# aidanmrli/rwm-pt-pytorch

Hardware: AMD Instinct MI355X
Metric: chain-MH-steps/sec (higher is better)
Workload: dtype f32; 1 GPU; BASELINE configs[2]: PT-RWM HIP, RoughCarpet dim=30 modes[-15,0,15], Normal proposal 2.38^2/dim, 32 geometric temps 1->0.01, swap_every=10, 65536 ladders per GPU; dim=30, temps=32, ladders_per_gpu=65536, mh_steps_per_launch=2000, swap_every=10, swap_mode=exchange, swap_order=sequential, rng=Philox4x32-10 in-kernel, world_size=1

## Files before the change

### rwm-pt-pytorch_amd/csrc/kernel.h

```cpp
#pragma once
#include <cstddef>
#include <type_traits>

#include "flow.h"
#include "philox.h"
#include "proposals.h"
#include "targets.h"

namespace ptrwm {

#ifndef PTRWM_BLOCK_THREADS
#define PTRWM_BLOCK_THREADS 256
#endif
constexpr int kBlockThreads = PTRWM_BLOCK_THREADS;
constexpr int kWavesPerBlock = kBlockThreads / 64;
struct StepLdsWords {
  static constexpr int kSwapWords = 3;
  static constexpr int kParkedInts = 3;
  static constexpr int kExtraPerThread = kSwapWords + kParkedInts + 2;
  static constexpr int kStreamSlabs = 2;
  static constexpr int kStreamStatPerThread = 5;
  static constexpr unsigned kVoteBytes = 16u;
  static constexpr unsigned kFlowLdsUnit = 8u;
  static constexpr int kFlowIntsPerThread = 4;
  static constexpr int kFlowUp = 2, kFlowDown = 3;
  static constexpr unsigned flow_bytes(int threads) { return (unsigned)(threads * kFlowIntsPerThread) * 4u; }
  static constexpr int floats_per_thread(int dp, bool stream) { return (stream ? kStreamSlabs * (dp + kStreamStatPerThread) : dp) + kExtraPerThread; }
  static constexpr unsigned bytes(int threads, int dp, bool stream, bool wide) { return (unsigned)(threads * floats_per_thread(dp, stream)) * 4u + (wide ? kVoteBytes : 0u); }
};
template <int DP, bool STREAM = false>
struct StepLds : StepLdsWords {
  static constexpr int kWaveFloats = 64 * floats_per_thread(DP, STREAM);
  static constexpr int kSlabFloats = 64 * DP;
  static constexpr int kSlabVectorsPerLane = (kSlabFloats + 255) / 256;
  static constexpr int s_l(int gt) { return STREAM ? kStreamSlabs * kSlabFloats : gt * DP; }
  static constexpr int parked(int gt) { return STREAM ? s_l(64) + kSwapWords * 64 : gt * (DP + kSwapWords); }
  static constexpr int sq_jump(int gt) { return STREAM ? s_l(64) + (kSwapWords + kParkedInts) * 64 : gt * (DP + (kSwapWords + kParkedInts)); }
  static constexpr int vote(int gt) { return gt * (DP + kExtraPerThread); }
  static constexpr int kSu = 1, kLanded = 2, kParked = kSwapWords, kVote = kExtraPerThread;
  static constexpr int kSwapCount = 1, kLastEvent = 2, kSqJump = kParkedInts;
  static constexpr int kZoneFloats = 64 * kStreamStatPerThread;
  static constexpr int zone(int slab) { return s_l(64) + 64 * kExtraPerThread + slab * kZoneFloats; }
  static constexpr int kZoneLogp = 0, kZoneSqJump = 64, kZoneAccept = 64 + 2 * 64;
  static constexpr int moments(bool wide, int gt) { return wide ? gt * (DP + kExtraPerThread) + (int)(kVoteBytes / 4u) : kBlockThreads * (DP + kExtraPerThread); }
  __device__ __forceinline__ static double *moments_region(float *s_dyn, bool wide, int gt, int wave, int stride) {
    return reinterpret_cast<double *>(s_dyn + moments(wide, gt)) + (wide ? 0 : wave * stride);
  }
  __device__ __forceinline__ static int *flow_region(float *s_dyn, bool wide, int wave, unsigned flow_lds) {
    return reinterpret_cast<int *>(s_dyn) + (int)flow_lds * (int)(kFlowLdsUnit / 4u) + (wide ? 0 : wave * (64 * kFlowIntsPerThread));
  }
  static constexpr unsigned bytes(int threads, bool wide) { return StepLdsWords::bytes(threads, DP, STREAM, wide); }
  static constexpr int kHeadWaveWords = normal_blocks(DP) * kHeadBlockSlots * kHeadSlotWords;
  static constexpr bool kHeadsFit = !STREAM && kHeadWaveWords <= 64 * (DP + kSwapWords) && kWaveFloats % kHeadSlotWords == 0;
  static constexpr int heads(bool wide, int wave) { return wave * (wide ? kHeadWaveWords : kWaveFloats); }
};
namespace lds_check {
using C = StepLds<30>;
using S = StepLds<30, true>;
static_assert(C::s_l(256) == 256 * 30 && C::parked(256) == C::s_l(256) + C::kParked * 256 &&
                  C::sq_jump(256) == C::parked(256) + C::kSqJump * 256 && C::vote(256) == C::sq_jump(256) + 2 * 256 &&
                  C::vote(256) == C::s_l(256) + C::kVote * 256 && C::moments(true, 256) * 4 == (int)C::bytes(256, true) &&
                  C::moments(false, 64) * 4 == (int)C::bytes(kBlockThreads, false) && C::kWaveFloats == C::vote(64) && 0 < C::kSu &&
                  C::kSu < C::kLanded && C::kLanded < C::kParked && 0 < C::kSwapCount && C::kSwapCount < C::kLastEvent && C::kLastEvent < C::kSqJump,
              "classic layout: rows, swap scratch, parked ints, squared-jump doubles, vote word, moments regions: disjoint, in this order");
static_assert(S::s_l(64) == 2 * S::kSlabFloats && S::parked(64) == S::s_l(64) + 3 * 64 && S::sq_jump(64) == S::parked(64) + 3 * 64 &&
                  S::zone(0) == S::sq_jump(64) + 2 * 64 && S::zone(1) == S::zone(0) + S::kZoneFloats &&
                  S::zone(1) + S::kZoneFloats == S::kWaveFloats && S::kZoneSqJump == S::kZoneLogp + 64 &&
                  S::kZoneAccept == S::kZoneSqJump + 2 * 64 && S::kZoneAccept + 2 * 64 == S::kZoneFloats,
              "streaming layout: two slabs, swap scratch, parked words, two landing zones of three arrays");
template <int DP>
constexpr bool aligned(bool ok = true) {
  using A = StepLds<DP>;
  using B = StepLds<DP, true>;
  for (int gt = 64; gt <= 256; gt += 64) ok = ok && A::sq_jump(gt) % 2 == 0 && A::moments(true, gt) % 2 == 0 && A::moments(false, gt) % 2 == 0;
  for (int z = 0; z < 2; ++z) ok = ok && B::zone(z) % 4 == 0 && (B::zone(z) + B::kZoneSqJump) % 4 == 0 && (B::zone(z) + B::kZoneAccept) % 4 == 0;
  return ok && A::kWaveFloats % 4 == 0 && B::kWaveFloats % 4 == 0 && B::kSlabFloats % 4 == 0 && B::sq_jump(64) % 2 == 0;
}
static_assert(aligned<2>() && aligned<3>() && aligned<5>() && aligned<9>() && aligned<29>() && aligned<30>() && aligned<50>() && aligned<64>(), "alignment");
static_assert(C::bytes(256, false) == 38912u && S::bytes(256, false) == 79872u && C::bytes(256, true) == 38928u, "LDS bytes, as before the layout had a name");
static_assert(C::kHeadsFit && C::kHeadWaveWords == 2048 && C::heads(false, 3) + C::kHeadWaveWords <= 3 * C::kWaveFloats + C::parked(64) &&
                  C::heads(true, 3) + C::kHeadWaveWords <= C::parked(256) && C::heads(true, 1) + C::kHeadWaveWords <= C::parked(128) &&
                  !StepLds<8>::kHeadsFit && !S::kHeadsFit,
              "parked heads: 16-byte slots over the rows and the swap scratch of the wave's group, below the parked words; width 8 has no room");
static_assert(0 < C::kFlowUp && C::kFlowUp < C::kFlowDown && C::kFlowDown < C::kFlowIntsPerThread && C::flow_bytes(256) == 4096u &&
                  C::flow_bytes(kBlockThreads) == (unsigned)kWavesPerBlock * 64u * C::kFlowIntsPerThread * 4u,
              "flow region: two word buffers, up visits, down visits, one region per group; nothing of it in a launch without flow");
}

constexpr int kNoStepInLaunch = (1 << 16) + 1;
struct FullArgs {
  const float *__restrict__ ext_prop;
  const float *__restrict__ ext_u;
  const float *__restrict__ ext_swap_u;
  float *__restrict__ trace;
  float *__restrict__ trace_logp;
  unsigned char *__restrict__ accept_flags;
  long long trace_chains;
  int trace_every;
  int mom_every;
  unsigned steps_to_trace : 17;
  unsigned trace_temps : 9;
  unsigned steps_to_mom : 17;
  unsigned mom_temps : 9;
  unsigned mom_chain : 1;
  double *__restrict__ mom_sum;
  double *__restrict__ mom_sum_sq;
  double *__restrict__ mom_sum_logp;
  long long *__restrict__ mom_count;
  int *__restrict__ flow_walker;
  long long *__restrict__ flow_round_trips;
  long long *__restrict__ flow_up;
  long long *__restrict__ flow_down;
};

typedef const __attribute__((address_space(4))) FullArgs *kargs_full_ptr;

struct KArgs {
  float *__restrict__ state;
  float *__restrict__ logp;
  const float *__restrict__ beta;
  const float *__restrict__ temp_scale;
  long long *__restrict__ n_accept;
  double *__restrict__ sq_jump;
  long long *__restrict__ swap_accept;
  long long *__restrict__ last_swap_ordinal;
  long long n_chains, chain_offset, step0;
  long long first_swap_event;
  int n_steps;
  int burn_left;
  int n_temps, dim, swap_every, swap_mode, swap_order, chains_per_wave;
  int steps_to_swap;
  unsigned k0, k1;
  unsigned full_mom_steps : 17;
  unsigned full_flow_lds : 15;
  TParams tp;
  PParams pp;
  FullArgs full;
};
static_assert(sizeof(FullArgs) == 136 && sizeof(KArgs) == 392 && offsetof(KArgs, tp) == 144, "the kernel arguments keep their size: see FullArgs");
static_assert(PTRWM_MAX_TEMPS < (1 << 9) && kNoStepInLaunch < (1 << 17) && 160u * 1024u / StepLdsWords::kFlowLdsUnit < (1u << 15), "FullArgs bitfield widths");
__host__ __device__ constexpr int ext_raw_per_step(int proposal_kind, int dim) { return dim + (proposal_kind == PTRWM_PROPOSAL_UNIFORM_RADIUS ? 1 : 0); }

__device__ __forceinline__ float swap_log_prob(float bj, float bk, float lj, float lk) {
  return sub_rn(sub_rn(add_rn(mul_rn(bj, lk), mul_rn(bk, lj)), mul_rn(bj, lj)), mul_rn(bk, lk));
}

__device__ __forceinline__ bool swap_accept_test(float u, float log_prob) {
  const float threshold = (log_prob >= 0.0f) ? 1.0f : hw_exp(log_prob);
  return u < threshold;
}

__device__ __forceinline__ bool mh_accept(float beta_t, float lp_new, float lp, float u_acc) {
  const float ratio = mul_rn(beta_t, sub_rn(lp_new, lp));
  return (ratio > 0.0f) || (u_acc < hw_exp(ratio));
}

__device__ __forceinline__ bool swap_pair_plain(int T, int t, float db, float lp, float us) {
  const bool last = t >= T - 1;
  const float u = last ? 0.5f : us;
  const float d = last ? 1.0f : db;
  const float inside = mul_rn(u, sub_rn(1.0f, u));
  return add_rn(__builtin_fminf(inside, d), mul_rn(lp, 0.0f)) > 0.0f;
}
__device__ __forceinline__ bool ladder_votes_plain(bool mine, int first_lane, int lanes_per_ladder) {
  const unsigned long long against = __builtin_amdgcn_ballot_w64(!mine);
  const unsigned long long ladder = (lanes_per_ladder >= 64 ? ~0ull : ((1ull << lanes_per_ladder) - 1ull)) << first_lane;
  return (against & ladder) == 0ull;
}

template <class Sync>
__device__ __forceinline__ bool wide_ladder_votes_plain(int *word, bool mine, int stamp, Sync sync) {
  if (!mine) *word = stamp;
  sync();
  return *word != stamp;
}

__device__ __forceinline__ float swap_uniform_ext(const float *__restrict__ ext_swap_u, long long event, long long n_chains,
                                                  long long chain, int T, int t) {
  return (t < T - 1) ? ext_swap_u[(event * n_chains + chain) * (T - 1) + t] : 2.0f;
}
__device__ __forceinline__ float swap_uniform_philox(uint32_t c0hi, uint32_t c1, uint32_t c2, uint32_t c3, uint32_t k0, uint32_t k1) {
  const u32x4 r = philox4x32_10(c0hi, c1, c2, c3, k0, k1);
  return u01(r.x);
}

#define PTRWM_SWAP_SCAN_PAIR(OK, IK, LK, LANDED_J, CAR_L, CAR_I) \
  do {                                                           \
    (LANDED_J) = (OK) ? (IK) : (CAR_I);                          \
    (CAR_L) = (OK) ? (CAR_L) : (LK);                             \
    (CAR_I) = (OK) ? (CAR_I) : (IK);                             \
  } while (0)

template <class Sync>
__device__ __forceinline__ void swap_decide(int T, int t, int base, int slot, int swap_mode, int swap_order, int par,
                                            const float *__restrict__ beta, float beta_t, float us, const float *s_l,
                                            float *s_u, int *landed, float &my_l, int &src, bool &pair_acc, Sync sync,
                                            bool plain) {
  if (swap_order == PTRWM_ORDER_SEQUENTIAL) {
    if (swap_mode == PTRWM_SWAP_EXCHANGE) {
      const bool has_k = t < T - 1;
      const float db = has_k ? sub_rn(beta_t, beta[t + 1]) : 1.0f;
      float car_l = s_l[base];
      int car_i = base;
      if (plain) {
        const float lk = s_l[has_k ? slot + 1 : slot];
        s_u[slot] = fmaf(-hw_ln(us), __builtin_amdgcn_rcpf(db), lk);
        sync();
#pragma unroll 2
        for (int j = 0; j < T - 1; ++j) {
          const int ik = base + j + 1;
          const float lkj = s_l[ik];
          const bool ok = car_l < s_u[base + j];
          PTRWM_SWAP_SCAN_PAIR(ok, ik, lkj, landed[base + j], car_l, car_i);
        }
      } else {
#pragma unroll 2
        for (int j = 0; j < T - 1; ++j) {
          const float lk = s_l[base + j + 1];
          const float u = s_u[base + j];
          const float bj = beta[j], bk = beta[j + 1];
          const bool ok = swap_accept_test(u, swap_log_prob(bj, bk, car_l, lk));
          const int ik = base + j + 1;
          PTRWM_SWAP_SCAN_PAIR(ok, ik, lk, landed[base + j], car_l, car_i);
        }
      }
      landed[base + T - 1] = car_i;
      src = landed[base + t];
      my_l = s_l[src];
      pair_acc = (t < T - 1) && (src == base + t + 1);
    } else {
      if (t < T - 1) {
        const float lk = s_l[slot + 1];
        const bool ok = swap_accept_test(us, swap_log_prob(beta_t, beta[t + 1], my_l, lk));
        if (ok) {
          my_l = lk;
          src = slot + 1;
        }
        pair_acc = ok;
      }
    }
  } else {
    const bool lower = ((t & 1) == par);
    const int partner_t = lower ? t + 1 : t - 1;
    const bool valid = partner_t >= 0 && partner_t < T;
    if (valid) {
      const int partner = base + partner_t;
      const float l_other = s_l[partner];
      const float u_low = lower ? us : s_u[partner];
      const int tj = lower ? t : partner_t;
      const float lj = lower ? my_l : l_other;
      const float lk = lower ? l_other : my_l;
      const bool ok = swap_accept_test(u_low, swap_log_prob(beta[tj], beta[tj + 1], lj, lk));
      if (ok && (lower || swap_mode == PTRWM_SWAP_EXCHANGE)) {
        my_l = l_other;
        src = partner;
      }
      pair_acc = ok && lower;
    }
  }
}

__device__ __forceinline__ int stage_head(const float *g) { return (int)((reinterpret_cast<uintptr_t>(g) >> 2) & 3u); }

template <bool LOAD>
__device__ __forceinline__ void stage_copy(float *__restrict__ lds, float *__restrict__ g, int total, int tid, int nthr) {
  typedef float vec4 __attribute__((ext_vector_type(4)));
  const int head = stage_head(g);
  vec4 *__restrict__ gv = reinterpret_cast<vec4 *>(g - head);
  vec4 *__restrict__ lv = reinterpret_cast<vec4 *>(lds);
  const int v_lo = head ? 1 : 0;
  const int v_hi = (head + total) >> 2;
  constexpr int kDepth = 4;
  int v0 = v_lo + tid;
  for (; v0 + (kDepth - 1) * nthr < v_hi; v0 += kDepth * nthr) {
    vec4 t[kDepth];
#pragma unroll
    for (int k = 0; k < kDepth; ++k) t[k] = LOAD ? gv[v0 + k * nthr] : lv[v0 + k * nthr];
#pragma unroll
    for (int k = 0; k < kDepth; ++k) (LOAD ? lv : gv)[v0 + k * nthr] = t[k];
  }
  if (v0 < v_hi) {
    vec4 t[kDepth - 1];
#pragma unroll
    for (int k = 0; k < kDepth - 1; ++k) {
      const int v = v0 + k * nthr;
      if (v < v_hi) t[k] = LOAD ? gv[v] : lv[v];
    }
#pragma unroll
    for (int k = 0; k < kDepth - 1; ++k) {
      const int v = v0 + k * nthr;
      if (v < v_hi) (LOAD ? lv : gv)[v] = t[k];
    }
  }
  const int e_lo = (4 * v_lo - head < total) ? 4 * v_lo - head : total;
  const int e_hi = (4 * v_hi - head > e_lo) ? 4 * v_hi - head : e_lo;
  if (tid < 6) {
    const int i = tid < 3 ? tid : e_hi + (tid - 3);
    const bool mine = tid < 3 ? (i < e_lo) : (i < total);
    if (mine) {
      if (LOAD) lds[head + i] = g[i];
      else g[i] = lds[head + i];
    }
  }
}

__device__ __forceinline__ int wave_in_block() { return __builtin_amdgcn_readfirstlane((int)(threadIdx.x >> 6)); }
__device__ __forceinline__ int thread_index_now(int wave) {
  unsigned all = ~0u;
  PTRWM_VALUE_BARRIER("+s"(all));
  return wave * 64 + (int)__builtin_amdgcn_mbcnt_hi(all, __builtin_amdgcn_mbcnt_lo(all, 0u));
}

__device__ __forceinline__ void count_add(long long *p, long long v) {
  (void)__hip_atomic_fetch_add(p, v, __ATOMIC_RELAXED, __HIP_MEMORY_SCOPE_AGENT);
}

constexpr unsigned moments_region_doubles(int rows, int dim) { return (unsigned)(rows * (2 * dim + 1)); }
constexpr int moments_rows(bool per_chain, int ladders_per_group, int temps) { return per_chain ? ladders_per_group * temps : temps; }

__device__ __forceinline__ void moments_add(double *p, double v) {
  (void)__hip_atomic_fetch_add(p, v, __ATOMIC_RELAXED, __HIP_MEMORY_SCOPE_WORKGROUP);
}

struct MomentsAcc {
  double *reg = nullptr;
  int temps, rows, dim;
  bool per_chain;
  struct Row { double *sum, *sum_sq, *logp; };

  template <class F>
  __device__ __forceinline__ MomentsAcc(F f, int ladders_per_group, int dim_)
      : temps(f->mom_temps), rows(moments_rows(f->mom_chain != 0, ladders_per_group, temps)), dim(dim_), per_chain(f->mom_chain != 0) {}
  __device__ __forceinline__ int doubles() const { return (int)moments_region_doubles(rows, dim); }
  __device__ __forceinline__ Row row(int cw, int t) const {
    const int r = per_chain ? cw * temps + t : t;
    return {reg + r * dim, reg + (rows + r) * dim, reg + 2 * rows * dim + r};
  }
  template <bool LOAD, class F>
  __device__ __forceinline__ void chain_copy(F f, int live_ladders, long long chain0, int tid, int nthr) const {
    const int live_rows = live_ladders * temps, n = live_rows * dim, rd = rows * dim;
    const long long row0 = chain0 * temps;
    double *const sum_logp = f->mom_sum_logp, *const gs = f->mom_sum + row0 * dim, *const gq = f->mom_sum_sq + row0 * dim;
    for (int i = tid; i < n; i += nthr) {
      if (LOAD) reg[i] = gs[i], reg[rd + i] = gq[i];
      else gs[i] = reg[i], gq[i] = reg[rd + i];
    }
    if (sum_logp != nullptr)
      for (int i = tid; i < live_rows; i += nthr) {
        if (LOAD) reg[2 * rd + i] = sum_logp[row0 + i];
        else sum_logp[row0 + i] = reg[2 * rd + i];
      }
  }
  template <class F>
  __device__ __forceinline__ void begin(F f, int live_ladders, long long chain0, int tid, int nthr) const {
    if (per_chain) chain_copy<true>(f, live_ladders, chain0, tid, nthr);
    else
      for (int i = tid; i < doubles(); i += nthr) reg[i] = 0.0;
  }
  template <class F>
  __device__ __forceinline__ void end(F f, long long mom_steps, long long live_ladders, long long chain0, int tid, int nthr) const {
    long long *const count = f->mom_count;
    if (per_chain) {
      chain_copy<false>(f, (int)live_ladders, chain0, tid, nthr);
      if (chain0 != 0) return;
    } else {
      const int td = temps * dim;
      double *const sum = f->mom_sum, *const sum_sq = f->mom_sum_sq, *const sum_logp = f->mom_sum_logp;
      const int n = 2 * td + (sum_logp != nullptr ? temps : 0);
      for (int i = tid; i < n; i += nthr) {
        const double v = reg[i];
        if (v != 0.0) unsafeAtomicAdd(i < td ? sum + i : (i < 2 * td ? sum_sq + (i - td) : sum_logp + (i - 2 * td)), v);
      }
    }
    const long long add = (per_chain ? 1 : live_ladders) * mom_steps;
    if (count != nullptr)
      for (int i = tid; i < temps; i += nthr) count_add(&count[i], add);
  }
};

__device__ __forceinline__ bool countdown_due(int &left, int period) {
  --left;
  const bool due = (left == 0);
  if (due) left = period;
  return due;
}

template <bool EXACT>
__device__ __forceinline__ int fresh_dim(int d0) {
  if constexpr (!EXACT) PTRWM_VALUE_BARRIER("+s"(d0));
  return d0;
}

typedef const __attribute__((address_space(4))) KArgs *kargs_ptr;
__device__ __forceinline__ kargs_ptr late_args() {
  uintptr_t p = (uintptr_t)__builtin_amdgcn_kernarg_segment_ptr();
  PTRWM_VALUE_BARRIER("+s"(p));
  return (kargs_ptr)p;
}

#ifndef PTRWM_J2_FENCE_MASK
#define PTRWM_J2_FENCE_MASK 7
#endif
#ifndef PTRWM_WAVES_SMALL
#define PTRWM_WAVES_SMALL 4
#endif
#ifndef PTRWM_WAVES_40
#define PTRWM_WAVES_40 3
#endif
#ifndef PTRWM_WAVES_MID
#define PTRWM_WAVES_MID 2
#endif
constexpr int min_waves_per_simd(int dp) {
  return dp <= 30 ? PTRWM_WAVES_SMALL : (dp <= 44 ? PTRWM_WAVES_40 : (dp <= 64 ? PTRWM_WAVES_MID : 1));
}
constexpr bool step_loop_at_register_cap(int dp, bool stream) { return !stream && min_waves_per_simd(dp) >= 4 && dp > 24; }

constexpr bool philox_heads_in_lds(int dp, bool exact, bool full, bool stream, int proposal_kind) {
  return !full && !stream && exact && dp == 30 && proposal_kind == PTRWM_PROPOSAL_NORMAL;
}

constexpr int stream_waves_per_simd(int dp) {
  return dp <= 10 ? 4 : (dp <= 20 ? 2 : (dp <= 30 ? 2 : 1));
}

constexpr int stream_register_waves(int dp) { return stream_waves_per_simd(dp) < 2 ? 2 : stream_waves_per_simd(dp); }

template <bool STREAM>
__device__ __forceinline__ int step_group_threads(int T) { return STREAM ? 64 : group_threads(T, 1); }

__device__ __forceinline__ long long step_replica_index(int i, long long n_chains, long long chain, int T, int t) {
  return ((long long)i * n_chains + chain) * T + t;
}
template <class F>
__device__ __forceinline__ const float *ext_prop_row(F f, int n_raw_ext, long long srep, int words) {
  return f->ext_prop + srep * n_raw_ext * words;
}
template <class F>
__device__ __forceinline__ long long trace_row_index(F f, int rows_written, long long chain, int t) {
  return ((long long)rows_written * f->trace_chains + chain) * (long long)f->trace_temps + t;
}

template <class Target, class Proposal, int DP, bool EXACT, bool FULL, bool STREAM = false>
__global__ void __launch_bounds__(kBlockThreads, STREAM ? stream_register_waves(DP) : min_waves_per_simd(DP)) ptrwm_step_kernel(const KArgs a) {
  static_assert(!(STREAM && FULL), "the streaming form is a production kernel: no fixture / trace arguments");
  const int T = a.n_temps;
  const int D0 = EXACT ? DP : a.dim;
  const int cpw = a.chains_per_wave;
  const bool wide = !STREAM && T > 64;
  const int wave = wave_in_block();
  const int tid = wide ? (int)threadIdx.x : (int)(threadIdx.x & 63);
  long long group = STREAM ? (long long)blockIdx.x * kWavesPerBlock + wave
                           : (wide ? (long long)blockIdx.x : (long long)blockIdx.x * kWavesPerBlock + (threadIdx.x >> 6));
  [[maybe_unused]] const long long n_groups = STREAM ? a.n_chains / cpw : 0;
  [[maybe_unused]] const long long group_stride = STREAM ? (long long)gridDim.x * kWavesPerBlock : 0;
  if (STREAM ? (group >= n_groups) : (group * cpw >= a.n_chains)) return;
  extern __shared__ __attribute__((aligned(16))) float s_dyn[];
  typedef float pf_vec4 __attribute__((ext_vector_type(4)));
  typedef StepLds<DP, STREAM> L;
  constexpr int NV = STREAM ? L::kSlabVectorsPerLane : 1;
  constexpr int kWaveFloats = L::kWaveFloats;
  [[maybe_unused]] int cur = 0;
  typedef const __attribute__((address_space(1))) void *dma_src;
  typedef __attribute__((address_space(3))) void *dma_dst;
  [[maybe_unused]] auto prefetch = [&](long long g, int slab) {
    const int tid = thread_index_now(wave) & 63;
    const kargs_ptr ap = late_args();
    const int n_vec = (cpw * T * D0) >> 2;
    const int n_live = cpw * T;
    float *const wbase = s_dyn + wave * kWaveFloats;
    const long long r0 = g * n_live;
    float *const zone = wbase + L::zone(slab);
    __builtin_amdgcn_global_load_lds((dma_src)(ap->logp + r0 + (tid < n_live ? tid : 0)), (dma_dst)(uintptr_t)(zone + L::kZoneLogp), 4, 0, 0);
    if (ap->sq_jump != nullptr && 2 * tid < n_live)
      __builtin_amdgcn_global_load_lds((dma_src)(ap->sq_jump + r0 + 2 * tid), (dma_dst)(uintptr_t)(zone + L::kZoneSqJump), 16, 0, 0);
    if (ap->n_accept != nullptr && 2 * tid < n_live)
      __builtin_amdgcn_global_load_lds((dma_src)(ap->n_accept + r0 + 2 * tid), (dma_dst)(uintptr_t)(zone + L::kZoneAccept), 16, 0, 0);
    const pf_vec4 *__restrict__ gv = reinterpret_cast<const pf_vec4 *>(ap->state + g * cpw * T * (long long)D0);
    float *const dst = wbase + slab * L::kSlabFloats;
#pragma unroll
    for (int k = 0; k < NV; ++k) {
      const int v = tid + 64 * k;
      if (v < n_vec) __builtin_amdgcn_global_load_lds((dma_src)(gv + v), (dma_dst)(uintptr_t)(dst + 256 * k), 16, 0, 0);
    }
  };
  [[maybe_unused]] float beta_t_s = 0.0f, tscale_s = 0.0f;
  [[maybe_unused]] float db_s = 1.0f;
  [[maybe_unused]] pf_vec4 pend_o[NV];
  [[maybe_unused]] float pend_lp = 0.0f;
  [[maybe_unused]] unsigned pend_n_swap = 0u;
  [[maybe_unused]] long long pend_acc = 0;
  [[maybe_unused]] bool pend_acc_on = false;
  [[maybe_unused]] double pend_sq = 0.0;
  [[maybe_unused]] long long pend_ord = 0, pend_group = 0;
  [[maybe_unused]] bool pend_sq_on = false, pend_ord_on = false, have_pending = false;
  [[maybe_unused]] auto flush_pending = [&]() {
    const kargs_ptr ap = late_args();
    const int tid = thread_index_now(wave) & 63;
    const int n_live = cpw * T;
    const int n_vec = (n_live * D0) >> 2;
    pf_vec4 *__restrict__ gv = reinterpret_cast<pf_vec4 *>(ap->state + pend_group * n_live * (long long)D0);
#pragma unroll
    for (int k = 0; k < NV; ++k) {
      const int v = tid + 64 * k;
      if (v < n_vec) gv[v] = pend_o[k];
    }
    if (tid < n_live) {
      const long long r = pend_group * n_live + tid;
      ap->logp[r] = pend_lp;
      if (pend_acc_on) ap->n_accept[r] = pend_acc;
      if (pend_sq_on) ap->sq_jump[r] = pend_sq;
      if (ap->swap_accept != nullptr && pend_n_swap != 0u) count_add(&ap->swap_accept[r], (long long)pend_n_swap);
      if (pend_ord_on) (void)__hip_atomic_fetch_max(&ap->last_swap_ordinal[r], pend_ord, __ATOMIC_RELAXED, __HIP_MEMORY_SCOPE_AGENT);
    }
  };
  if constexpr (STREAM) {
    const int cw_s = tid / T;
    const int t_s = cw_s < cpw ? tid - cw_s * T : 0;
    beta_t_s = a.beta[t_s];
    tscale_s = a.temp_scale[t_s];
    db_s = sub_rn(beta_t_s, a.beta[t_s < T - 1 ? t_s + 1 : t_s]);
    prefetch(group, 0);
  }
  do {
  const long long chain0 = group * cpw;
  const int cw_raw = tid / T;
  const int t_raw = tid - cw_raw * T;
  const bool live = (cw_raw < cpw) && (chain0 + cw_raw < a.n_chains);
  const int cw = live ? cw_raw : 0;
  const int t = live ? t_raw : 0;
  const long long chain = chain0 + cw;
  const long long rep = chain0 * T + (live ? tid : 0);

  float *const s_stage = STREAM ? s_dyn + wave * kWaveFloats + cur * L::kSlabFloats
                                : s_dyn + (wide ? 0 : (int)(threadIdx.x >> 6) * kWaveFloats);
  auto sync_group = [&]() {
    if (wide) {
      __syncthreads();
    } else {
      __builtin_amdgcn_fence(__ATOMIC_ACQ_REL, "wavefront");
      __builtin_amdgcn_wave_barrier();
    }
  };

  float x[DP], y[DP];
  {
    const long long live_chains = (a.n_chains - chain0 < cpw) ? (a.n_chains - chain0) : cpw;
    const int stage_total = (int)live_chains * T * D0;
    float *__restrict__ gs = a.state + chain0 * T * (long long)D0;
    const int nthr = step_group_threads<STREAM>(T);
    int row_head = 0;
    if constexpr (!STREAM) {
      stage_copy<true>(s_stage, gs, stage_total, tid, nthr);
      row_head = stage_head(gs);
      if (wide) reinterpret_cast<int *>(s_dyn)[L::vote(nthr)] = 0;
      if constexpr (FULL) {
        if (a.full.mom_sum != nullptr) {
          MomentsAcc m(&a.full, cpw, D0);
          m.reg = L::moments_region(s_dyn, wide, nthr, wave, m.doubles());
          m.begin(&a.full, (int)live_chains, chain0, tid, nthr);
        }
        if (a.full.flow_walker != nullptr) {
          int *const fl = L::flow_region(s_dyn, wide, wave, a.full_flow_lds) + tid;
          fl[0] = live ? a.full.flow_walker[rep] : 0;
          fl[L::kFlowUp * nthr] = 0;
          fl[L::kFlowDown * nthr] = 0;
        }
      }
    }
    if constexpr (STREAM) asm volatile("s_waitcnt vmcnt(0)" ::: "memory");
    sync_group();
    const float *row = s_stage + row_head + (live ? tid : 0) * D0;
#pragma unroll
    for (int d = 0; d < DP; ++d) x[d] = (d < D0) ? row[d] : 0.0f;
  }
  float lp;
  [[maybe_unused]] double sq_old = 0.0;
  [[maybe_unused]] long long acc_old = 0;
  if constexpr (STREAM) {
    {
      const float *zone = s_dyn + wave * kWaveFloats + L::zone(cur);
      lp = (zone + L::kZoneLogp)[tid];
      if (a.sq_jump != nullptr) sq_old = reinterpret_cast<const double *>(zone + L::kZoneSqJump)[tid < cpw * T ? tid : 0];
      if (a.n_accept != nullptr) acc_old = reinterpret_cast<const long long *>(zone + L::kZoneAccept)[tid < cpw * T ? tid : 0];
    }
    if (have_pending) flush_pending();
    if (group + group_stride < n_groups) prefetch(group + group_stride, cur ^ 1);
  } else {
    lp = a.logp[rep];
  }
  const float beta_t = STREAM ? beta_t_s : a.beta[t];
  const float tscale = STREAM ? tscale_s : a.temp_scale[t];
  bool jump_trusted = false;
  if constexpr (Proposal::kKnowsJump) {
    float xmax = 0.0f;
#pragma unroll
    for (int d = 0; d < DP; ++d) xmax = __builtin_fmaxf(xmax, __builtin_fabsf(x[d]));
    jump_trusted = xmax <= kJumpTrust * Proposal::increment_scale(tscale, a.pp);
  }

  const unsigned long long gchain = (unsigned long long)(a.chain_offset + chain);
  constexpr bool kHeads = philox_heads_in_lds(DP, EXACT, FULL, STREAM, Proposal::kKind);
  static_assert(!kHeads || L::kHeadsFit, "the parked heads need room over the rows and the swap scratch");
  typename std::conditional<kHeads, RngCtxHeads, RngCtx>::type rc;
  rc.c2 = chain_word_c2(gchain);
  rc.k0 = a.k0;
  rc.k1 = a.k1;
  const uint32_t c3_base = chain_word_c3(gchain, (uint32_t)t);
  [[maybe_unused]] auto head_slot0 = [&]() __attribute__((always_inline)) {
    return reinterpret_cast<PhiloxHeadSlot *>(s_dyn + L::heads(wide, wave)) + (thread_index_now(wave) & 63);
  };
  [[maybe_unused]] auto store_heads = [&](uint32_t c0hi, uint32_t c3) __attribute__((always_inline)) {
    PhiloxHeadSlot *const slot0 = head_slot0();
    uint32_t chain_hi, chain_lo;
    philox_mul(kPhiloxM1, rc.c2, chain_hi, chain_lo);
#pragma unroll
    for (int c = 0; c < normal_blocks(DP); ++c) {
      const PhiloxHead h = philox_head(c0hi | (uint32_t)c, chain_lo, c3, rc.k0, rc.k1);
      slot0[c * kHeadBlockSlots] = PhiloxHeadSlot{h.pk, h.qk, h.ql, 0u};
    }
  };
  if constexpr (kHeads) {
    sync_group();
    store_heads(step_word_c0hi((unsigned long long)a.step0), with_stream(c3_base, kStreamMH));
  }

  unsigned n_acc = 0;
  {
    const int gt = step_group_threads<STREAM>(T);
    int *const park = reinterpret_cast<int *>(STREAM ? s_dyn + wave * kWaveFloats + L::parked(gt) : s_stage + L::parked(gt)) + tid;
    park[0] = (int)c3_base;
    park[L::kSwapCount * gt] = 0;
    park[L::kLastEvent * gt] = -1;
    reinterpret_cast<double *>(park - tid + L::kSqJump * gt)[tid] = 0.0;
  }

  const bool ext = FULL && a.full.ext_prop != nullptr;
  const bool trace_on =
      FULL && live && a.full.trace != nullptr && (chain < a.full.trace_chains) && (t < (int)a.full.trace_temps);
  int to_swap = a.steps_to_swap;
  int to_trace = FULL ? (int)a.full.steps_to_trace : 0;
  [[maybe_unused]] int to_mom = FULL ? (int)a.full.steps_to_mom : 0;
  int trace_rows = 0;
  int swap_in_call = 0;
  const int ev_par0 = (int)(a.first_swap_event & 1);
  unsigned long long s = (unsigned long long)a.step0;

  constexpr int W = canon_width(DP);
  auto commit_plain = [&](bool acc, float jump, int jump_kind, int D) __attribute__((always_inline)) -> float {
    float j2;
    if (jump_kind != kJumpNone) {
      float from_states = 0.0f;
      if (!jump_trusted) {
        PTRWM_COLD_PATH();
        float j2p[4] = {0.0f, 0.0f, 0.0f, 0.0f};
        PTRWM_DIM_LOOP(d, DP, D, {
          const float dl = sub_rn(y[d], x[d]);
          j2p[d / W] = fmaf(dl, dl, j2p[d / W]);
        })
        from_states = tree4_add(j2p);
      }
      PTRWM_DIM_LOOP(d, DP, D, {
        x[d] = acc ? y[d] : x[d];
        if ((d & PTRWM_J2_FENCE_MASK) == PTRWM_J2_FENCE_MASK) sched_fence_soft();
      })
      j2 = acc ? (jump_trusted ? jump : from_states) : 0.0f;
    } else {
      float j2p[4] = {0.0f, 0.0f, 0.0f, 0.0f};
      PTRWM_DIM_LOOP(d, DP, D, {
        const float dl = sub_rn(y[d], x[d]);
        j2p[d / W] = fmaf(dl, dl, j2p[d / W]);
        x[d] = acc ? y[d] : x[d];
        if ((d & PTRWM_J2_FENCE_MASK) == PTRWM_J2_FENCE_MASK) sched_fence_soft();
      })
      j2 = tree4_add(j2p);
      if (!acc) j2 = 0.0f;
    }
    return j2;
  };
  auto finish_step = [&](bool count_on, bool acc, float j2, int D) __attribute__((always_inline)) {
    if (count_on) {
      n_acc += acc ? 1u : 0u;
      const int tid_q = thread_index_now(wave);
      const int gt_q = wide ? group_threads(T, 1) : 64;
      double *const sq_slot = reinterpret_cast<double *>(
                                  STREAM ? s_dyn + wave * kWaveFloats + L::sq_jump(64)
                                         : s_dyn + (wide ? 0 : wave * kWaveFloats) + L::sq_jump(gt_q)) +
                              (wide ? tid_q : (tid_q & 63));
      (void)__hip_atomic_fetch_add(sq_slot, (double)j2, __ATOMIC_RELAXED, __HIP_MEMORY_SCOPE_WAVEFRONT);
    }
    if constexpr (FULL) {
      const bool trace_now = a.full.trace != nullptr && countdown_due(to_trace, a.full.trace_every);
      if (trace_now && trace_on) {
        const long long row = trace_row_index(&a.full, trace_rows, chain, t);
        float *__restrict__ tr = a.full.trace + row * D;
        PTRWM_DIM_LOOP(d, DP, D, { tr[d] = x[d]; })
        if (a.full.trace_logp != nullptr) a.full.trace_logp[row] = lp;
      }
      trace_rows += trace_now ? 1 : 0;
      if (a.full.mom_sum != nullptr && countdown_due(to_mom, a.full.mom_every) && count_on && live && t < (int)a.full.mom_temps) {
        MomentsAcc m(&a.full, cpw, D);
        m.reg = L::moments_region(s_dyn, wide, step_group_threads<STREAM>(T), wave, m.doubles());
        const MomentsAcc::Row r = m.row(cw, t);
        PTRWM_DIM_LOOP(d, DP, D, {
          const double v = (double)x[d];
          moments_add(r.sum + d, v);
          moments_add(r.sum_sq + d, v * v);
        })
        moments_add(r.logp, (double)lp);
      }
    }
  };

  int i = 0;
  while (i < a.n_steps) {
    const int left = a.n_steps - i;
    const bool to_multiple = to_swap <= left;
    int run = to_multiple ? to_swap : left;
    to_swap = to_multiple ? a.swap_every : to_swap - left;
    bool count_on, acc;
    float lp_mh;
    float jump;
    int jump_kind;
    int D;
    for (;; ++i, ++s) {
      count_on = i >= a.burn_left;
      rc.c0hi = step_word_c0hi(s);
      rc.c1 = step_word_c1(s);
      rc.c3 = with_stream(c3_base, kStreamMH);
      if constexpr (step_loop_at_register_cap(DP, STREAM) && !kHeads) asm volatile("" : "+v"(rc.c2));
      if constexpr (kHeads) rc.heads = head_slot0();

      long long srep = 0;
      const float *ext_raw = nullptr;
      float ext_u = 0.0f;
      if constexpr (FULL) {
        srep = step_replica_index(i, a.n_chains, chain, T, t);
        if (ext) {
          ext_raw = ext_prop_row(&a.full, ext_raw_per_step(Proposal::kKind, D0), srep, 1);
          ext_u = a.full.ext_u[srep];
        }
      }

      jump = 0.0f;
      const float u_acc = Proposal::propose(y, x, fresh_dim<EXACT>(D0), tscale, a.pp, rc, ext_raw, ext_u, jump, jump_kind);
      const float lp_new = Target::template logp<false>(y, fresh_dim<EXACT>(D0), a.tp);
      D = fresh_dim<EXACT>(D0);

      acc = mh_accept(beta_t, lp_new, lp, u_acc);
      lp_mh = acc ? lp_new : lp;
      if constexpr (FULL) {
        if (a.full.accept_flags != nullptr && live) a.full.accept_flags[srep] = acc ? 1 : 0;
      }

      if (--run == 0) break;
      const float j2 = commit_plain(acc, jump, jump_kind, D);
      lp = lp_mh;
      finish_step(count_on, acc, j2, D);
    }
    const bool swap_due = to_multiple && count_on && (T > 1);

    float j2;
    if (!swap_due) {
      j2 = commit_plain(acc, jump, jump_kind, D);
      lp = lp_mh;
    } else {
      const int tid_s = thread_index_now(wave);
      const int slot = wide ? tid_s : (tid_s & 63);
      const int group_threads = step_group_threads<STREAM>(T);
      float *const rows = STREAM ? s_dyn + wave * kWaveFloats + cur * L::kSlabFloats
                                 : s_dyn + (wide ? 0 : (tid_s >> 6) * kWaveFloats);
      float *const s_l = STREAM ? s_dyn + wave * kWaveFloats + L::s_l(64) : rows + L::s_l(group_threads);
      float *const s_u = s_l + L::kSu * group_threads;
      int *const park = reinterpret_cast<int *>(s_l + L::kParked * group_threads) + slot;
      const uint32_t c3_s = (uint32_t)park[0];
      const int t = temperature_of(c3_s);
      const int base = live ? slot - t : 0;
      int src = slot;
      float my_l = lp_mh;
      bool pair_acc = false;
      float us;
      if (ext) us = swap_uniform_ext(a.full.ext_swap_u, swap_in_call, a.n_chains, chain, T, t);
      else us = swap_uniform_philox(rc.c0hi, rc.c1, rc.c2, with_stream(c3_s, kStreamSwap), rc.k0, rc.k1);
      if constexpr (kHeads) sync_group();
      s_l[slot] = my_l;
      s_u[slot] = us;
      const bool pair_plain = swap_pair_plain(T, t, STREAM ? db_s : sub_rn(beta_t, a.beta[t < T - 1 ? t + 1 : t]), my_l, us);
      bool swap_plain;
      if (wide) {
        swap_plain = wide_ladder_votes_plain(reinterpret_cast<int *>(s_l + L::kVote * group_threads), pair_plain, swap_in_call + 1, sync_group);
      } else {
        swap_plain = ladder_votes_plain(pair_plain, base, T);
        sync_group();
      }
      swap_decide(T, t, base, slot, a.swap_mode, a.swap_order, (ev_par0 + swap_in_call) & 1, a.beta, beta_t, us, s_l, s_u,
                  reinterpret_cast<int *>(s_u + (L::kLanded - L::kSu) * group_threads), my_l, src, pair_acc, sync_group, swap_plain);
      if (pair_acc) {
        park[L::kSwapCount * group_threads] += 1;
        park[L::kLastEvent * group_threads] = swap_in_call;
      }
      {
        float j2p[4] = {0.0f, 0.0f, 0.0f, 0.0f};
        float *my_row = rows + slot * D;
        PTRWM_DIM_LOOP(d, DP, D, { my_row[d] = acc ? y[d] : x[d]; })
        sync_group();
        const int Dr = fresh_dim<EXACT>(D0);
        const float *src_row = rows + src * Dr;
        PTRWM_DIM_LOOP(d, DP, Dr, {
          const float w = src_row[d];
          const float dl = sub_rn(w, x[d]);
          j2p[d / W] = fmaf(dl, dl, j2p[d / W]);
          x[d] = w;
          if ((d & 7) == 7) sched_fence_soft();
        })
        j2 = tree4_add(j2p);
        if constexpr (kHeads) {
          sync_group();
          store_heads(rc.c0hi, with_stream(c3_s, kStreamMH));
        }
        if constexpr (FULL) {
          if (a.full.flow_walker != nullptr && live) {
            int *const fl = L::flow_region(s_dyn, wide, wave, a.full_flow_lds);
            const int buf = swap_in_call & 1;
            bool trip;
            const int32_t fw = flow_ends(fl[buf * group_threads + src], t, T, trip);
            fl[(buf ^ 1) * group_threads + slot] = fw;
            if (trip && flow_id(fw) < T && a.full.flow_round_trips != nullptr) {
              long long ch = chain;
              PTRWM_VALUE_BARRIER("+v"(ch));
              a.full.flow_round_trips[ch * T + flow_id(fw)] += 1;
            }
            fl[L::kFlowUp * group_threads + slot] += (int)flow_visit_up(fw);
            fl[L::kFlowDown * group_threads + slot] += (int)flow_visit_down(fw);
          }
        }
      }
      lp = my_l;
      ++swap_in_call;
    }
    finish_step(count_on, acc, j2, D);
    ++i;
    ++s;
  }

  const kargs_ptr ae = late_args();
  long long c0_out;
  {
    const int T2 = fresh_dim<false>(T), D2 = EXACT ? DP : fresh_dim<false>(D0), cpw2 = fresh_dim<false>(cpw);
    const bool wide2 = T2 > 64;
    const int tx2 = thread_index_now(wave);
    const int tid2 = wide2 ? tx2 : (tx2 & 63);
    float *const rows2 = STREAM ? s_dyn + wave * kWaveFloats + cur * L::kSlabFloats : s_dyn + (wide2 ? 0 : wave * kWaveFloats);
    long long c0;
    if constexpr (STREAM) {
      c0 = group * cpw2;
    } else {
      const long long bid = (long long)fresh_dim<false>((int)blockIdx.x);
      c0 = (wide2 ? bid : bid * kWavesPerBlock + wave) * cpw2;
    }
    const long long n_chains2 = ae->n_chains;
    const long long live_chains = (n_chains2 - c0 < cpw2) ? (n_chains2 - c0) : cpw2;
    const int stage_total = (int)live_chains * T2 * D2;
    const long long stage_g0 = c0 * T2 * (long long)D2;
    c0_out = c0;
    float *__restrict__ gs = ae->state + stage_g0;
    sync_group();
    if (live) {
      float *row = rows2 + stage_head(gs) + tid2 * D2;
#pragma unroll
      for (int d = 0; d < DP; ++d)
        if (d < D2) row[d] = x[d];
    }
    sync_group();
    const int nthr = group_threads(T2, 1);
    if constexpr (FULL) {
      const kargs_full_ptr fa = &ae->full;
      if (fa->mom_sum != nullptr) {
        MomentsAcc m(fa, cpw2, D2);
        m.reg = L::moments_region(s_dyn, wide2, nthr, wave, m.doubles());
        m.end(fa, (long long)ae->full_mom_steps, live_chains, c0, tid2, nthr);
      }
    }
    if constexpr (STREAM) {
      const pf_vec4 *__restrict__ lv = reinterpret_cast<const pf_vec4 *>(rows2);
      const int n_vec = stage_total >> 2;
#pragma unroll
      for (int k = 0; k < NV; ++k) {
        const int v = tid2 + 64 * k;
        if (v < n_vec) pend_o[k] = lv[v];
      }
    } else {
      stage_copy<false>(rows2, gs, stage_total, tid2, nthr);
    }
  }
  if (live) {
    const int tid_o = thread_index_now(wave);
    const int T_o = fresh_dim<false>(T);
    const long long rep = c0_out * T_o + (T_o > 64 ? tid_o : (tid_o & 63));
    const int gt_o = group_threads(T_o, 1);
    const int *const park = reinterpret_cast<const int *>(STREAM ? s_dyn + wave * kWaveFloats + L::parked(64)
                                                                 : s_dyn + (T_o > 64 ? 0 : (tid_o >> 6) * kWaveFloats) + L::parked(gt_o)) +
                            (T_o > 64 ? tid_o : (tid_o & 63));
    const int t = temperature_of((uint32_t)park[0]);
    const unsigned n_swap_acc = (unsigned)park[L::kSwapCount * gt_o];
    const int last_event = park[L::kLastEvent * gt_o];
    const int tid_g = T_o > 64 ? tid_o : (tid_o & 63);
    const double sq = reinterpret_cast<const double *>(park - tid_g + L::kSqJump * gt_o)[tid_g];
    if constexpr (STREAM) {
      pend_lp = lp;
      pend_acc_on = ae->n_accept != nullptr && n_acc != 0u;
      pend_acc = acc_old + (long long)n_acc;
      pend_n_swap = n_swap_acc;
      pend_sq_on = ae->sq_jump != nullptr && sq != 0.0;
      pend_sq = sq_old + sq;
      pend_ord_on = ae->last_swap_ordinal != nullptr && last_event >= 0;
      const long long ev = ae->first_swap_event + last_event;
      pend_ord = swap_attempt_ordinal(ae->swap_order, ev, T_o, t);
    } else {
    ae->logp[rep] = lp;
    if (ae->n_accept != nullptr && n_acc != 0u) count_add(&ae->n_accept[rep], (long long)n_acc);
    if (ae->sq_jump != nullptr && sq != 0.0) ae->sq_jump[rep] += sq;
    if (ae->swap_accept != nullptr && n_swap_acc != 0u) count_add(&ae->swap_accept[rep], (long long)n_swap_acc);
    if (ae->last_swap_ordinal != nullptr && last_event >= 0) {
      const long long ev = ae->first_swap_event + last_event;
      const long long ord = swap_attempt_ordinal(ae->swap_order, ev, T_o, t);
      if (ord > ae->last_swap_ordinal[rep]) ae->last_swap_ordinal[rep] = ord;
    }
    if constexpr (FULL) {
      const kargs_full_ptr fa = &ae->full;
      if (fa->flow_walker != nullptr) {
        const int *const fl = L::flow_region(s_dyn, T_o > 64, wave, ae->full_flow_lds) + tid_g;
        fa->flow_walker[rep] = fl[(swap_in_call & 1) * gt_o];
        const int n_up = fl[L::kFlowUp * gt_o], n_down = fl[L::kFlowDown * gt_o];
        if (fa->flow_up != nullptr && n_up != 0) count_add(&fa->flow_up[rep], (long long)n_up);
        if (fa->flow_down != nullptr && n_down != 0) count_add(&fa->flow_down[rep], (long long)n_down);
      }
    }
    }
  }
  if constexpr (!STREAM) break;
  pend_group = group;
  have_pending = true;
  group += group_stride;
  cur ^= 1;
  } while (group < n_groups);
  if constexpr (STREAM) flush_pending();
}

template <class Target, int DP>
__global__ void __launch_bounds__(kBlockThreads) ptrwm_logdensity_kernel(const float *__restrict__ x,
                                                                          float *__restrict__ out,
                                                                          long long n, int D, TParams tp) {
  const long long i = (long long)blockIdx.x * kBlockThreads + threadIdx.x;
  if (i >= n) return;
  float y[DP];
  const float *__restrict__ xp = x + i * D;
#pragma unroll
  for (int d = 0; d < DP; ++d) y[d] = (d < D) ? xp[d] : 0.0f;
  out[i] = Target::template logp<true>(y, D, tp);
}

constexpr int standalone_min_waves(int dp) { return dp > 64 ? 2 : 1; }

template <class Proposal, int DP>
__global__ void __launch_bounds__(kBlockThreads, standalone_min_waves(DP)) ptrwm_propose_kernel(
    float *__restrict__ out, long long n, int D, int T, const float *__restrict__ temp_scale, PParams pp,
    const float *__restrict__ ext_raw, int n_raw_ext, unsigned k0, unsigned k1) {
  const long long i = (long long)blockIdx.x * kBlockThreads + threadIdx.x;
  if (i >= n * T) return;
  const long long row = i / T;
  const int t = (int)(i - row * T);
  float x[DP], y[DP];
#pragma unroll
  for (int d = 0; d < DP; ++d) x[d] = 0.0f;
  RngCtx rc;
  rc.c0hi = step_word_c0hi((unsigned long long)row);
  rc.c1 = step_word_c1((unsigned long long)row);
  rc.c2 = chain_word_c2(0ull);
  rc.c3 = with_stream(chain_word_c3(0ull, (uint32_t)t), kStreamMH);
  rc.k0 = k0;
  rc.k1 = k1;
  const float *er = ext_raw != nullptr ? ext_raw + i * n_raw_ext : nullptr;
  float jump = 0.0f;
  int jump_kind;
  Proposal::propose(y, x, D, temp_scale[t], pp, rc, er, 0.0f, jump, jump_kind);
  float *__restrict__ op = out + i * D;
#pragma unroll
  for (int d = 0; d < DP; ++d)
    if (d < D) op[d] = y[d];
}

constexpr unsigned split_tile_lds_bytes(int dim) { return (unsigned)(64 * dim + 4) * 4u; }

template <class Proposal, int DP>
__global__ void __launch_bounds__(64, standalone_min_waves(DP)) ptrwm_split_propose_kernel(
    const float *__restrict__ state, float *__restrict__ proposals, float *__restrict__ accept_u, long long n_chains,
    long long chain_offset, unsigned long long step, int D, int T, const float *__restrict__ temp_scale, PParams pp,
    const float *__restrict__ ext_raw, const float *__restrict__ ext_u, int n_raw_ext, unsigned k0, unsigned k1,
    const long long *__restrict__ device_step) {
  extern __shared__ __attribute__((aligned(16))) float s_tile[];
  const int lane = (int)threadIdx.x;
  const long long n_reps = n_chains * T;
  const long long first = (long long)blockIdx.x * 64;
  if (first >= n_reps) return;
  if (device_step != nullptr) step += (unsigned long long)*device_step;
  const int n_rows = (n_reps - first < 64) ? (int)(n_reps - first) : 64;
  const bool live = lane < n_rows;
  const long long i = first + (live ? lane : 0);
  const long long chain = i / T;
  const int t = (int)(i - chain * T);
  float x[DP], y[DP];
  float *__restrict__ gx = const_cast<float *>(state) + first * D;
  stage_copy<true>(s_tile, gx, n_rows * D, lane, 64);
  __builtin_amdgcn_fence(__ATOMIC_ACQ_REL, "wavefront");
  __builtin_amdgcn_wave_barrier();
  {
    const float *row = s_tile + stage_head(gx) + (live ? lane : 0) * D;
#pragma unroll
    for (int d = 0; d < DP; ++d) x[d] = (d < D) ? row[d] : 0.0f;
  }
  const unsigned long long gchain = (unsigned long long)(chain_offset + chain);
  RngCtx rc;
  rc.c0hi = step_word_c0hi(step);
  rc.c1 = step_word_c1(step);
  rc.c2 = chain_word_c2(gchain);
  rc.c3 = with_stream(chain_word_c3(gchain, (uint32_t)t), kStreamMH);
  rc.k0 = k0;
  rc.k1 = k1;
  const float *er = ext_raw != nullptr ? ext_raw + i * n_raw_ext : nullptr;
  float jump = 0.0f;
  int jump_kind;
  const float u = Proposal::propose(y, x, D, temp_scale[t], pp, rc, er, ext_u != nullptr ? ext_u[i] : 0.0f, jump, jump_kind);
  float *__restrict__ gy = proposals + first * D;
  __builtin_amdgcn_fence(__ATOMIC_ACQ_REL, "wavefront");
  __builtin_amdgcn_wave_barrier();
  if (live) {
    float *row = s_tile + stage_head(gy) + lane * D;
#pragma unroll
    for (int d = 0; d < DP; ++d)
      if (d < D) row[d] = y[d];
  }
  __builtin_amdgcn_fence(__ATOMIC_ACQ_REL, "wavefront");
  __builtin_amdgcn_wave_barrier();
  stage_copy<false>(s_tile, gy, n_rows * D, lane, 64);
  if (!live) return;
  accept_u[i] = u;
  float xmax = 0.0f;
#pragma unroll
  for (int d = 0; d < DP; ++d) xmax = __builtin_fmaxf(xmax, __builtin_fabsf(x[d]));
  const bool trusted = Proposal::kKnowsJump && xmax <= kJumpTrust * Proposal::increment_scale(temp_scale[t], pp);
  accept_u[n_reps + i] = (jump_kind == kJumpTotal && trusted) ? jump : -1.0f;
}

}
```

Before: 48.82 billion chain-MH-steps/s.

## Replace sequential swap scan with wave-ballot bitmask walk for exchange swaps

For sequential exchange swaps with dim up to 44 and non-wide ladders, each thread's serial scan over the ladder is replaced by a wave-level walk. At every pair step one ballot collects which carriers pass, and bitmask arithmetic advances the carrier and records rejections for all ladders in the wave at once. Each thread then finds its source slot with a count-leading-zeros lookup, so the per-thread landed array writes and the dependent LDS reads of the carried log-probability disappear. It adds a ballot per pair step and a cold path for non-plain tests. It also assumes ladders are packed inside one 64-lane wave.

```diff
diff --git a/rwm-pt-pytorch_amd/csrc/kernel.h b/rwm-pt-pytorch_amd/csrc/kernel.h
--- a/rwm-pt-pytorch_amd/csrc/kernel.h
+++ b/rwm-pt-pytorch_amd/csrc/kernel.h
@@ -5,6 +5,7 @@
 #include "flow.h"
 #include "philox.h"
 #include "proposals.h"
+#include "swap_walk.h"
 #include "targets.h"
 
 namespace ptrwm {
@@ -191,13 +192,14 @@
     (CAR_I) = (OK) ? (CAR_I) : (IK);                             \
   } while (0)
 
-template <class Sync>
+template <bool SCAN = true, class Sync>
 __device__ __forceinline__ void swap_decide(int T, int t, int base, int slot, int swap_mode, int swap_order, int par,
                                             const float *__restrict__ beta, float beta_t, float us, const float *s_l,
                                             float *s_u, int *landed, float &my_l, int &src, bool &pair_acc, Sync sync,
                                             bool plain) {
   if (swap_order == PTRWM_ORDER_SEQUENTIAL) {
     if (swap_mode == PTRWM_SWAP_EXCHANGE) {
+      if constexpr (!SCAN) return;
       const bool has_k = t < T - 1;
       const float db = has_k ? sub_rn(beta_t, beta[t + 1]) : 1.0f;
       float car_l = s_l[base];
@@ -260,6 +262,43 @@
   }
 }
 
+template <bool LEAN, class Sync>
+__device__ __forceinline__ void swap_walk_decide(int T, int t, int base, int slot, const float *__restrict__ beta, float db,
+                                                 float us, const float *s_l, float *s_u, float &my_l, int &src, bool &pair_acc,
+                                                 Sync sync, bool plain) {
+  const bool has_k = t < T - 1;
+  if (plain) {
+    const float lk = s_l[has_k ? slot + 1 : slot];
+    s_u[slot] = fmaf(-hw_ln(us), __builtin_amdgcn_rcpf(db), lk);
+  }
+  sync();
+  const uint64_t seg0 = __builtin_amdgcn_ballot_w64(slot == base);
+  const float *const pair = s_u + base;
+  const bool all_plain = __builtin_amdgcn_ballot_w64(!plain) == 0ull;
+  SwapWalk w = swap_walk_begin(seg0);
+  int j = 0;
+  if constexpr (!LEAN) {
+    if (all_plain)
+      for (; j + 2 <= T - 1; j += 2) {
+        swap_walk_step(w, seg0, j, __builtin_amdgcn_ballot_w64(my_l < pair[j]));
+        swap_walk_step(w, seg0, j + 1, __builtin_amdgcn_ballot_w64(my_l < pair[j + 1]));
+      }
+  }
+#pragma unroll 1
+  for (; j < T - 1; ++j) {
+    const float v = pair[j];
+    bool ok = my_l < v;
+    if (!all_plain) {
+      PTRWM_COLD_PATH();
+      const bool literal = swap_accept_test(v, swap_log_prob(beta[j], beta[j + 1], my_l, s_l[base + j + 1]));
+      ok = plain ? ok : literal;
+    }
+    swap_walk_step(w, seg0, j, __builtin_amdgcn_ballot_w64(ok));
+  }
+  src = swap_walk_source(w.rejected, seg0, base + t, has_k, pair_acc);
+  my_l = s_l[src];
+}
+
 __device__ __forceinline__ int stage_head(const float *g) { return (int)((reinterpret_cast<uintptr_t>(g) >> 2) & 3u); }
 
 template <bool LOAD>
@@ -424,6 +463,8 @@
 }
 
 constexpr int stream_register_waves(int dp) { return stream_waves_per_simd(dp) < 2 ? 2 : stream_waves_per_simd(dp); }
+
+constexpr bool swap_walk_in_kernel(int dp) { return dp <= 44; }
 
 template <bool STREAM>
 __device__ __forceinline__ int step_group_threads(int T) { return STREAM ? 64 : group_threads(T, 1); }
@@ -784,7 +825,8 @@
       if constexpr (kHeads) sync_group();
       s_l[slot] = my_l;
       s_u[slot] = us;
-      const bool pair_plain = swap_pair_plain(T, t, STREAM ? db_s : sub_rn(beta_t, a.beta[t < T - 1 ? t + 1 : t]), my_l, us);
+      const float db_pair = STREAM ? db_s : sub_rn(beta_t, a.beta[t < T - 1 ? t + 1 : t]);
+      const bool pair_plain = swap_pair_plain(T, t, db_pair, my_l, us);
       bool swap_plain;
       if (wide) {
         swap_plain = wide_ladder_votes_plain(reinterpret_cast<int *>(s_l + L::kVote * group_threads), pair_plain, swap_in_call + 1, sync_group);
@@ -792,8 +834,11 @@
         swap_plain = ladder_votes_plain(pair_plain, base, T);
         sync_group();
       }
-      swap_decide(T, t, base, slot, a.swap_mode, a.swap_order, (ev_par0 + swap_in_call) & 1, a.beta, beta_t, us, s_l, s_u,
-                  reinterpret_cast<int *>(s_u + (L::kLanded - L::kSu) * group_threads), my_l, src, pair_acc, sync_group, swap_plain);
+      if (swap_walk_in_kernel(DP) && !wide && a.swap_order == PTRWM_ORDER_SEQUENTIAL && a.swap_mode == PTRWM_SWAP_EXCHANGE)
+        swap_walk_decide<FULL>(T, t, base, slot, a.beta, db_pair, us, s_l, s_u, my_l, src, pair_acc, sync_group, swap_plain);
+      else
+        swap_decide<!(STREAM && swap_walk_in_kernel(DP))>(T, t, base, slot, a.swap_mode, a.swap_order, (ev_par0 + swap_in_call) & 1, a.beta, beta_t, us, s_l, s_u,
+                    reinterpret_cast<int *>(s_u + (L::kLanded - L::kSu) * group_threads), my_l, src, pair_acc, sync_group, swap_plain);
       if (pair_acc) {
         park[L::kSwapCount * group_threads] += 1;
         park[L::kLastEvent * group_threads] = swap_in_call;
diff --git a/rwm-pt-pytorch_amd/csrc/swap_walk.h b/rwm-pt-pytorch_amd/csrc/swap_walk.h
--- /dev/null
+++ b/rwm-pt-pytorch_amd/csrc/swap_walk.h
@@ -0,0 +1,35 @@
+#pragma once
+#include <stdint.h>
+
+#ifndef PTRWM_HD
+#ifdef __HIPCC__
+#define PTRWM_HD __host__ __device__
+#else
+#define PTRWM_HD
+#endif
+#endif
+
+namespace ptrwm {
+
+struct SwapWalk {
+  uint64_t carrier, rejected;
+};
+
+PTRWM_HD inline SwapWalk swap_walk_begin(uint64_t seg0) { return SwapWalk{seg0, 0ull}; }
+
+PTRWM_HD inline void swap_walk_step(SwapWalk &w, uint64_t seg0, int j, uint64_t pass) {
+  const uint64_t next = seg0 << (j + 1);
+  const uint64_t failed = w.carrier & ~pass;
+  const uint64_t fresh = (failed + (next - seg0)) & next;
+  w.carrier = (w.carrier & pass) | fresh;
+  w.rejected |= fresh;
+}
+
+PTRWM_HD inline int swap_walk_source(uint64_t rejected, uint64_t seg0, int pos, bool has_pair, bool &pair_acc) {
+  pair_acc = has_pair && ((rejected >> pos) & 2ull) == 0ull;
+  const uint64_t upto = (2ull << pos) - 1ull;
+  const int carrier = 63 - __builtin_clzll(((rejected | seg0) & upto) | 1ull);
+  return pair_acc ? pos + 1 : carrier;
+}
+
+}
```

Result: faster. 49.40 billion chain-MH-steps/s, median of 6 (+1.2%).
